# kahrendt/esp-audio-libs

Measured on NVIDIA B200. Metric: resampled output Msamples/s (4096 stereo streams, 256 taps), higher is better.
Workload: dtype f32

## Files before the change

esp-audio-libs_b200/csrc/kernels.hpp:

```cpp
#pragma once
#include <cuda.h>
#include <cuda_runtime.h>
#include <stddef.h>
#include <stdint.h>

#include "common.hpp"

namespace espb {

void count_launch();

struct PerDeviceOnce {
  bool done[64] = {};
  bool first() {
    int dev = 0;
    if (cudaGetDevice(&dev) != cudaSuccess || dev < 0 || dev >= 64)
      return true;
    const bool was = done[dev];
    done[dev] = true;
    return !was;
  }
};

struct ResampleParams {
  const float *xt;
  int64_t xt_rows;
  float *out;
  int64_t out_ss, out_cs, out_fs;
  float *out_tm;
  int64_t out_tm_rows;
  const float *G;
  const ChunkEntry *chunks;
  const int32_t *pass_chunk_begin;
  const OutEntry *outs;
  int n_series, channels, n_out, taps;
  int pass_first, pass_end, passes_per_cta, g_chunk_base;
  int out_vec;
  const int *ready;
  int ready_tiles, ready_target;
};
constexpr int kReadyTileRows = 32;
struct DirectInput {
  const float *in;
  int64_t in_ss;
  alignas(64) CUtensorMap map;
};
struct ResampleDirectParams {
  ResampleParams p;
  DirectInput d;
};
enum OutVec : int { kOutVecNone = 0, kOutVecPlanar = 1, kOutVecStereo = 2, kOutVecFrame4 = 3, kOutVecTimeMajor = 4 };

size_t resample_smem_bytes(int bpp, int chunk_rows, int g_row_floats = kGRowFloats);
size_t g_chunk_floats(int bpp, int chunk_rows, int g_row_floats = kGRowFloats);
cudaError_t launch_finalize(OutEntry *outs, int n, int n_filters, bool lowpass, bool interp, cudaStream_t stream);
cudaError_t launch_expand_schedule(const SchedSegment *segs, int n_segs, OutEntry *outs, int n, int n_filters,
                                   bool lowpass, bool interp, cudaStream_t stream);
cudaError_t launch_expand(const float *bank, const OutEntry *outs, const ChunkEntry *chunks, float *G,
                          int chunk_first, int n_chunks, int n_out, int taps, int bpp, int chunk_rows,
                          bool split_at_zero, cudaStream_t stream, int g_row_floats = kGRowFloats);
cudaError_t launch_resample(const ResampleParams &p, int bpp, int chunk_rows, bool exact, cudaStream_t stream,
                            const DirectInput *direct = nullptr, bool non_interpolating = false);
cudaError_t launch_resample_ni(const ResampleParams &q, int n_groups, int n_ctas_y, bool exact, bool tm,
                               cudaStream_t stream);
cudaError_t launch_resample_direct(const ResampleParams &p, const DirectInput &d, int n_groups, int n_ctas_y,
                                   bool exact, cudaStream_t stream);
cudaError_t launch_transpose(const float *in, int64_t in_ss, int64_t in_cs, int64_t in_fs, int channels, int n_series,
                             int n_in, float *xt, int64_t rows_cap, int row_first, int pad_rows,
                             cudaStream_t stream);
cudaError_t launch_transpose_flags(const float *in, int64_t in_ss, int64_t in_cs, int64_t in_fs, int channels,
                                   int n_series, int n_in, float *xt, int64_t rows_cap, int row_first, int pad_rows,
                                   int *ready, int ctas_per_sm, cudaStream_t stream, int *n_tiles);

struct FsGroupDesc {
  int64_t x_off;
  int64_t x_old_off;
  int64_t out_off;
  int64_t in_off;
  int32_t n_in, n_out;
  int32_t outs_begin;
  int32_t seg_begin, n_segs;
  int32_t carry_row;
};
cudaError_t launch_stage_small(const float *old_xt, int carry_row, int taps, const float *in, int64_t in_ss,
                               int64_t in_cs, int64_t in_fs, int channels, int n_series, int n_in, float *xt,
                               int64_t rows_cap, int pad_rows, cudaStream_t stream);
cudaError_t launch_transpose_ptrs(const float *const *planes_dev, int n_series, int n_in, float *xt, int64_t rows_cap,
                                  int row_first, int pad_rows, cudaStream_t stream);
cudaError_t launch_untranspose_ptrs(const float *tm, int64_t rows_cap, int row_first, int n_rows,
                                    float *const *planes_dev, int n_series, cudaStream_t stream);

struct FsParams {
  const float *x;
  int64_t x_fs;
  int x_row0;
  float *out;
  int64_t out_ss, out_cs, out_fs;
  float *out_tm;
  const float *bank_tr;
  const OutEntry *outs;
  int n_series, channels, n_out, taps;
  int kt, slice_floats;
  int q_per_out, x_tile_floats, out_vec, x_pitch, stages;
  const FsGroupDesc *groups;
};
struct FsGeometry {
  int sv, b, q;
  int outputs_per_cta;
};
constexpr int kFsMaxSeries = 32;
int fs_slice_taps(int taps, int filters);
size_t fs_slice_floats(int filters, int kt);
void fs_build_bank_slices(const float *bank, int taps, int filters, int kt, float *dst);
FsGeometry fs_geometry(int n_series);
size_t fs_smem_bytes(const FsGeometry &g, size_t slice_floats, int x_rows);
cudaError_t launch_resample_fs(const FsParams &p, const FsGeometry &g, int x_rows, bool exact, cudaStream_t stream,
                               int n_groups = 1);
cudaError_t launch_fsg_stage(const FsGroupDesc *groups, int n_groups, const float *old_buf, float *new_buf, int pitch,
                             int taps, const float *in, int64_t in_ss, int channels, int n_series, int max_rows,
                             cudaStream_t stream);
cudaError_t launch_expand_schedule_groups(const FsGroupDesc *groups, int n_groups, const SchedSegment *segs,
                                          OutEntry *outs, int max_n_out, int n_filters, bool lowpass, bool interp,
                                          cudaStream_t stream);

cudaError_t launch_q2f(const uint8_t *in, int64_t in_row_bytes, float *out, int64_t out_row_floats, int rows,
                       uint32_t row_samples, int bits, float gain_factor, cudaStream_t stream);
cudaError_t launch_f2q(const float *in, int64_t in_row_floats, uint8_t *out, int64_t out_row_bytes, int rows,
                       uint32_t row_samples, int bits, uint32_t *clipped, bool clipped_per_row, cudaStream_t stream);

int launch_pcm_to_tm(const uint8_t *in, int64_t in_row_bytes, int bits, float gain_factor, int channels, int n_series,
                     int n_frames, float *tm, int64_t rows_cap, int row_first, cudaStream_t stream, cudaError_t *err);
int launch_tm_to_pcm(const float *tm, int64_t rows_cap, int row_first, int n_frames, uint8_t *out,
                     int64_t out_row_bytes, int bits, int channels, int n_series, uint32_t *clipped_per_stream,
                     cudaStream_t stream, cudaError_t *err);
cudaError_t launch_transpose_from(const float *in, int64_t in_ss, int64_t in_cs, int64_t in_fs, int channels,
                                  int n_series, int n_in, float *xt, int64_t rows_cap, int row_first, int j_begin,
                                  int pad_rows, cudaStream_t stream);
cudaError_t launch_untranspose_from(const float *tm, int64_t rows_cap, int row_first, int j_begin, int n_rows,
                                    float *out, int64_t out_ss, int64_t out_cs, int64_t out_fs, int channels,
                                    int n_series, cudaStream_t stream);

struct BiquadParams {
  float a0, a1, a2, b1, b2;
  int first_order;
};
size_t biquad_block_state_floats(int n_series, int n_sections, int n_rows, int block_rows);
constexpr int kBiquadFewSeries = 32;
cudaError_t launch_biquad_cl(float *buf, int64_t ss, int64_t cs, int64_t fs, int channels, int n_series, int n_frames,
                             int n_sections, BiquadParams c, float *state, cudaStream_t stream);
cudaError_t launch_biquad_tm(const float *src, float *dst, int64_t rows_cap, int row_first, int n_rows, int n_series,
                             int n_sections, BiquadParams c, float *state ,
                             int block_rows, int warm_rows, cudaStream_t stream, float *blk_state = nullptr,
                             unsigned int *mismatches = nullptr, unsigned int *chain_broken = nullptr);
int launch_biquad_tm_pcm(float *buf, int64_t rows_cap, int row_first, int n_rows, int n_series, int n_sections,
                         BiquadParams c, float *state, uint8_t *out, int64_t out_row_bytes, int bits,
                         uint32_t *clipped_per_stream, cudaStream_t stream, cudaError_t *err);
cudaError_t launch_untranspose(const float *tm, int64_t rows_cap, int row_first, int n_rows, float *out,
                               int64_t out_ss, int64_t out_cs, int64_t out_fs, int channels, int n_series,
                               cudaStream_t stream);

cudaError_t launch_add_s16(const int16_t *a, const int16_t *b, int16_t *out, uint64_t n, int64_t s1, int64_t s2,
                           int64_t so, int shift, cudaStream_t stream);
cudaError_t launch_mulc_s16(const int16_t *a, int16_t *out, uint64_t n, int16_t c, int64_t si, int64_t so,
                            cudaStream_t stream);

cudaError_t launch_checksum(const uint32_t *words, uint64_t n, unsigned long long *sum_dev, cudaStream_t stream);
cudaError_t run_tile_probe(double *tflops);
cudaError_t run_fma_probe(double *tflops, double *clock_mhz, double *tflops_scalar, double *tflops_packed);

}
```

esp-audio-libs_b200/csrc/resample_device.cuh:

```cuda
#pragma once
#include <cuda.h>
#include <cuda_runtime.h>
#include <stdint.h>

#include "common.hpp"
#include "kernels.hpp"

namespace espb {
namespace {

constexpr int NB = kOutputsPerBlock;
constexpr int SGN = kSeriesPerRow;
constexpr uint32_t kPassDone = 1u << 9, kHistory = 1u << 10;
constexpr int RG = 4;

__device__ __forceinline__ uint32_t smem_u32(const void *p) { return (uint32_t) __cvta_generic_to_shared(p); }

__device__ __forceinline__ void mbar_init(uint64_t *bar, int count) {
  asm volatile("mbarrier.init.shared::cta.b64 [%0], %1;\n" ::"r"(smem_u32(bar)), "r"(count) : "memory");
}
__device__ __forceinline__ void mbar_expect_tx(uint64_t *bar, uint32_t bytes) {
  asm volatile("mbarrier.arrive.expect_tx.shared::cta.b64 _, [%0], %1;\n" ::"r"(smem_u32(bar)), "r"(bytes)
               : "memory");
}
__device__ __forceinline__ void mbar_wait(uint64_t *bar, uint32_t parity) {
  const uint32_t a = smem_u32(bar);
  asm volatile(
      "{\n"
      ".reg .pred p;\n"
      "WAIT_%=:\n"
      "mbarrier.try_wait.parity.shared::cta.b64 p, [%0], %1;\n"
      "@p bra DONE_%=;\n"
      "bra WAIT_%=;\n"
      "DONE_%=:\n"
      "}\n" ::"r"(a),
      "r"(parity)
      : "memory");
}
__device__ __forceinline__ void tma_bulk_g2s(void *dst_smem, const void *src, uint32_t bytes, uint64_t *bar) {
  asm volatile("cp.async.bulk.shared::cluster.global.mbarrier::complete_tx::bytes [%0], [%1], %2, [%3];\n" ::"r"(
                   smem_u32(dst_smem)),
               "l"(src), "r"(bytes), "r"(smem_u32(bar))
               : "memory");
}

__device__ __forceinline__ void tma_tensor2d_g2s(void *dst_smem, const CUtensorMap *map, int c0, int c1, uint64_t *bar) {
  asm volatile(
      "cp.async.bulk.tensor.2d.shared::cluster.global.tile.mbarrier::complete_tx::bytes [%0], [%1, {%2, %3}], [%4];\n" ::"r"(
          smem_u32(dst_smem)),
      "l"(map), "r"(c0), "r"(c1), "r"(smem_u32(bar))
      : "memory");
}

__device__ __forceinline__ void cp_async_16(void *dst_smem, const void *src) {
  asm volatile("cp.async.ca.shared.global [%0], [%1], 16;\n" ::"r"(smem_u32(dst_smem)), "l"(src) : "memory");
}
__device__ __forceinline__ void cp_async_wait_all() { asm volatile("cp.async.wait_all;\n" ::: "memory"); }

struct SwzTile {
  float *p;
  __device__ __forceinline__ static int unit(int row, int u) { return u ^ (((row >> 2) ^ ((row & 3) << 3)) & 31); }
  __device__ __forceinline__ float &at(int row, int col) const {
    return p[row * kSeriesPerRow + (unit(row, col >> 2) << 2) + (col & 3)];
  }
  __device__ __forceinline__ float4 &vec(int row, int u) const {
    return *reinterpret_cast<float4 *>(p + row * kSeriesPerRow + (unit(row, u) << 2));
  }
};

__device__ __forceinline__ int ld_acquire_gpu(const int *p) {
  int v;
  asm volatile("ld.acquire.gpu.global.s32 %0, [%1];\n" : "=r"(v) : "l"(p) : "memory");
  return v;
}
__device__ __forceinline__ void fence_proxy_async() { asm volatile("fence.proxy.async;\n" ::: "memory"); }
__device__ __forceinline__ void grid_launch_dependents() { asm volatile("griddepcontrol.launch_dependents;\n" ::: "memory"); }

__device__ __forceinline__ uint64_t l2_policy_evict_first() {
  uint64_t pol;
  asm volatile("createpolicy.fractional.L2::evict_first.b64 %0, 1.0;\n" : "=l"(pol));
  return pol;
}
__device__ __forceinline__ uint64_t l2_policy_evict_last() {
  uint64_t pol;
  asm volatile("createpolicy.fractional.L2::evict_last.b64 %0, 1.0;\n" : "=l"(pol));
  return pol;
}
__device__ __forceinline__ float4 ld_global_hint(const float4 *p, uint64_t pol) {
  float4 v;
  asm volatile("ld.global.nc.L1::no_allocate.L2::cache_hint.v4.f32 {%0, %1, %2, %3}, [%4], %5;\n"
               : "=f"(v.x), "=f"(v.y), "=f"(v.z), "=f"(v.w)
               : "l"(p), "l"(pol));
  return v;
}
__device__ __forceinline__ void st_global_hint(float4 *p, float4 v, uint64_t pol) {
  asm volatile("st.global.L2::cache_hint.v4.f32 [%0], {%1, %2, %3, %4}, %5;\n" ::"l"(p), "f"(v.x), "f"(v.y), "f"(v.z),
               "f"(v.w), "l"(pol)
               : "memory");
}
__device__ __forceinline__ void tma_bulk_g2s_hint(void *dst_smem, const void *src, uint32_t bytes, uint64_t *bar,
                                                  uint64_t pol) {
  asm volatile(
      "cp.async.bulk.shared::cluster.global.mbarrier::complete_tx::bytes.L2::cache_hint [%0], [%1], %2, [%3], %4;\n" ::"r"(
          smem_u32(dst_smem)),
      "l"(src), "r"(bytes), "r"(smem_u32(bar)), "l"(pol)
      : "memory");
}

__device__ __forceinline__ int smem_arrive(int *counter) {
  int old;
  asm volatile("atom.relaxed.cta.shared::cta.add.s32 %0, [%1], 1;\n" : "=r"(old) : "r"(smem_u32(counter)) : "memory");
  return old;
}

__device__ __forceinline__ float2 fma2(float2 g, float x, float2 acc) {
  return __ffma2_rn(g, make_float2(x, x), acc);
}

template <bool EXACT>
__device__ __forceinline__ float mac(float g, float x, float acc) {
  if (EXACT)
    return __fadd_rn(acc, __fmul_rn(g, x));
  return __fmaf_rn(g, x, acc);
}

}
}
```

esp-audio-libs_b200/csrc/resample_direct_kernel.cu:

```cuda
#include <cuda.h>
#include <cuda_runtime.h>
#include <stdint.h>
#include <stdio.h>
#include <stdlib.h>

#include "common.hpp"
#include "kernels.hpp"
#include "resample_device.cuh"

namespace espb {

template <int BPP, int NST, int CJ, bool EXACT, bool TMCAP, bool DIRECT>
__device__ __forceinline__ void resample_body(const ResampleParams &p, const DirectInput &din, unsigned char *smem_raw) {
  static_assert(!DIRECT || (CJ == 32 && !TMCAP), "direct input: 32-row chunks, caller-layout output");
  constexpr int NTHREADS = BPP * 32;
  constexpr int STAGES = NST;
  constexpr int MAXC = max_chunks_per_cta(BPP, CJ);
  static_assert(kMaxPassesPerCta * BPP * sizeof(int2) <= (size_t) NST * CJ * SGN * sizeof(float), "set-up table");
  constexpr int XS_STAGE = CJ * SGN;
  constexpr int GS_STAGE = CJ * BPP * kGRowFloats;
  constexpr uint32_t X_BYTES = XS_STAGE * sizeof(float), G_BYTES = GS_STAGE * sizeof(float);

  float *gs = reinterpret_cast<float *>(smem_raw);
  float *xs = gs + STAGES * GS_STAGE;
  uint64_t *full = reinterpret_cast<uint64_t *>(xs + STAGES * XS_STAGE);
  int *done = reinterpret_cast<int *>(full + STAGES);
  int32_t *jtab = reinterpret_cast<int32_t *>(done + 2 * STAGES);
  uint16_t *rtab = reinterpret_cast<uint16_t *>(jtab + MAXC);
  OutEntry *etab = reinterpret_cast<OutEntry *>(rtab + MAXC * BPP);
  int32_t *hdr = reinterpret_cast<int32_t *>(etab + BPP * NB);
  int2 *wtab = reinterpret_cast<int2 *>(smem_raw);

  const int tid = threadIdx.x, lane = tid & 31, warp = tid >> 5;
  const int group = blockIdx.x;
  const int T = p.taps;

  const int pass_first = p.pass_first + blockIdx.y * p.passes_per_cta;
  int pass_last = pass_first + p.passes_per_cta;
  if (pass_last > p.pass_end)
    pass_last = p.pass_end;
  const int chunk_first = p.pass_chunk_begin[pass_first], chunk_last = p.pass_chunk_begin[pass_last];
  const int n_chunks = __shfl_sync(0xffffffffu, chunk_last - chunk_first, 0);

  for (int i = tid; i < (pass_last - pass_first) * BPP; i += NTHREADS) {
    const int o0 = ((pass_first + i / BPP) * BPP + (i % BPP)) * NB;
    int2 w = make_int2(0, 0);
    if (o0 < p.n_out) {
      const int o1 = (o0 + NB <= p.n_out ? o0 + NB : p.n_out) - 1;
      w.x = p.outs[o0].ws;
      w.y = p.outs[o1].ws + T;
    }
    wtab[i] = w;
  }
  if (tid == 0) {
#pragma unroll
    for (int s = 0; s < STAGES; ++s) {
      mbar_init(&full[s], 1);
      done[s] = 0;
    }
    hdr[0] = chunk_first - p.g_chunk_base;
    asm volatile("fence.mbarrier_init.release.cluster;\n" ::: "memory");
  }
  __syncthreads();
  for (int i = tid; i < n_chunks; i += NTHREADS) {
    const ChunkEntry ce = p.chunks[chunk_first + i];
    const bool last_of_pass = (i + 1 == n_chunks) || (p.chunks[chunk_first + i + 1].pass != ce.pass);
    jtab[i] = ce.j_start;
#pragma unroll
    for (int w = 0; w < BPP; ++w) {
      const int2 win = wtab[(ce.pass - pass_first) * BPP + w];
      int r0 = win.x - ce.j_start, r1 = win.y - ce.j_start;
      r0 = r0 < 0 ? 0 : (r0 / RG);
      r1 = r1 > CJ ? CJ / RG : ((r1 + RG - 1) / RG);
      if (r0 > CJ / RG)
        r0 = CJ / RG;
      if (r1 < r0)
        r1 = r0;
      if (DIRECT && ce.j_start < 0) {
        const int lim = (-ce.j_start) / RG;
        r1 = r1 < lim ? r1 : lim;
        r0 = r0 < r1 ? r0 : r1;
      }
      rtab[i * BPP + w] = (uint16_t) (r0 | (r1 << 4) | (last_of_pass ? kPassDone : 0) |
                                      ((DIRECT && ce.j_start < 0) ? kHistory : 0));
    }
  }
  __syncthreads();

  auto issue_chunk = [&](int c) {
    const int st = c % STAGES;
    const float *xt_group = p.xt + (int64_t) blockIdx.x * p.xt_rows * SGN;
    mbar_expect_tx(&full[st], X_BYTES + G_BYTES);
    tma_bulk_g2s(gs + st * GS_STAGE, p.G + (size_t) (hdr[0] + c) * GS_STAGE, G_BYTES, &full[st]);
    const int j = jtab[c];
    if (DIRECT && j >= 0) {
      tma_tensor2d_g2s(xs + st * XS_STAGE, &din.map, 2 * j, (int) blockIdx.x * (SGN / 2), &full[st]);
      tma_tensor2d_g2s(xs + st * XS_STAGE + XS_STAGE / 2, &din.map, 2 * j + 32, (int) blockIdx.x * (SGN / 2), &full[st]);
    } else {
      tma_bulk_g2s(xs + st * XS_STAGE, xt_group + (int64_t) (j + T) * SGN, X_BYTES, &full[st]);
    }
  };
  if (tid == 0)
    for (int c = 0; c < STAGES && c < n_chunks; ++c)
      issue_chunk(c);

  float2 acc2[EXACT ? 1 : 4][EXACT ? 1 : NB];
  float acc1[EXACT ? 4 : 1][EXACT ? NB : 1][2];
  auto clear_acc = [&]() {
    if constexpr (EXACT) {
#pragma unroll
      for (int e = 0; e < 4; ++e)
#pragma unroll
        for (int n = 0; n < NB; ++n)
          acc1[e][n][0] = acc1[e][n][1] = 0.0f;
    } else {
#pragma unroll
      for (int e = 0; e < 4; ++e)
#pragma unroll
        for (int n = 0; n < NB; ++n)
          acc2[e][n] = make_float2(0.0f, 0.0f);
    }
  };
  clear_acc();

  int cur_pass = pass_first;
  uint32_t role_next = rtab[warp];
  for (int c = 0; c < n_chunks; ++c) {
    const int st = c % STAGES;
    const uint32_t role = role_next;
    const bool pass_done = (role & kPassDone) != 0;
    const int r0 = role & 15, r1 = (role >> 4) & 15;
    if (pass_done && lane < NB) {
      int o = (cur_pass * BPP + warp) * NB + lane;
      o = o < p.n_out ? o : p.n_out - 1;
      cp_async_16(&etab[warp * NB + lane], &p.outs[o]);
    }
    mbar_wait(&full[st], (uint32_t) ((c / STAGES) & 1));
    if constexpr (!DIRECT)
    {
      const float *xrow = xs + st * XS_STAGE + lane * 4;
      const float *grow = gs + st * GS_STAGE + warp * kGRowFloats;
      for (int jb = r0; jb < r1; ++jb) {
        const float *xb = xrow + jb * RG * SGN;
        const float *gb = grow + jb * RG * BPP * kGRowFloats;
#pragma unroll
        for (int jj = 0; jj < RG; ++jj) {
          const float4 xv = *reinterpret_cast<const float4 *>(xb + jj * SGN);
          if constexpr (EXACT) {
            const float4 *gp = reinterpret_cast<const float4 *>(gb + jj * BPP * kGRowFloats);
            const float4 g0 = gp[0], g1 = gp[1], g2 = gp[2], g3 = gp[3];
            const float x4[4] = {xv.x, xv.y, xv.z, xv.w};
            const float g16[16] = {g0.x, g0.y, g0.z, g0.w, g1.x, g1.y, g1.z, g1.w,
                                   g2.x, g2.y, g2.z, g2.w, g3.x, g3.y, g3.z, g3.w};
#pragma unroll
            for (int n = 0; n < NB; ++n)
#pragma unroll
              for (int e = 0; e < 4; ++e) {
                acc1[e][n][0] = mac<true>(g16[2 * n], x4[e], acc1[e][n][0]);
                acc1[e][n][1] = mac<true>(g16[2 * n + 1], x4[e], acc1[e][n][1]);
              }
          } else {
            const float4 *gp = reinterpret_cast<const float4 *>(gb + jj * BPP * kGRowFloats);
            const float4 g0 = gp[0], g1 = gp[1], g2 = gp[2], g3 = gp[3];
            const float x4[4] = {xv.x, xv.y, xv.z, xv.w};
            const float2 gg[NB] = {make_float2(g0.x, g0.y), make_float2(g0.z, g0.w), make_float2(g1.x, g1.y),
                                   make_float2(g1.z, g1.w), make_float2(g2.x, g2.y), make_float2(g2.z, g2.w),
                                   make_float2(g3.x, g3.y), make_float2(g3.z, g3.w)};
#pragma unroll
            for (int n = 0; n < NB; ++n)
#pragma unroll
              for (int e = 0; e < 4; ++e)
                acc2[e][n] = fma2(gg[n], x4[e], acc2[e][n]);
          }
        }
      }
    }
    else
    {
      auto row_update = [&](const float (&x4)[4], const float *grow_j) {
        const float4 *gp = reinterpret_cast<const float4 *>(grow_j);
        const float4 g0 = gp[0], g1 = gp[1], g2 = gp[2], g3 = gp[3];
        if constexpr (EXACT) {
          const float g16[16] = {g0.x, g0.y, g0.z, g0.w, g1.x, g1.y, g1.z, g1.w,
                                 g2.x, g2.y, g2.z, g2.w, g3.x, g3.y, g3.z, g3.w};
#pragma unroll
          for (int n = 0; n < NB; ++n)
#pragma unroll
            for (int e = 0; e < 4; ++e) {
              acc1[e][n][0] = mac<true>(g16[2 * n], x4[e], acc1[e][n][0]);
              acc1[e][n][1] = mac<true>(g16[2 * n + 1], x4[e], acc1[e][n][1]);
            }
        } else {
          const float2 gg[NB] = {make_float2(g0.x, g0.y), make_float2(g0.z, g0.w), make_float2(g1.x, g1.y),
// ... 195 lines not shown
```

esp-audio-libs_b200/csrc/resample_kernel.cu:

```cuda
#include <cuda_runtime.h>
#include <stdint.h>
#include <stdio.h>
#include <stdlib.h>

#include "common.hpp"
#include "kernels.hpp"
#include "resample_device.cuh"

namespace espb {


__global__ void __launch_bounds__(256)
    espb_finalize_kernel(OutEntry *__restrict__ outs, int n, float n_filters, int lowpass, int interp) {
  const int k = blockIdx.x * blockDim.x + threadIdx.x;
  if (k >= n)
    return;
  const float off = outs[k].w;
  const float fl = (float) (int) off;
  float frac = __fsub_rn(off, fl);
  OutEntry e;
  e.ws = outs[k].ws + (int32_t) fl;
  e.phase = 0;
  e.w = 0.0f;
  if (frac == 0.0f && !lowpass) {
// ... 327 lines not shown
                              float *__restrict__ xt, int64_t rows_cap, int row_first, int pad_rows) {
  __shared__ float tile[TR_ROWS][SGN + 1];
  const int g = blockIdx.x;
  const int j0 = blockIdx.y * TR_ROWS;
  const int tid = threadIdx.x;
  const int total_rows = n_in + pad_rows;
  for (int i = tid; i < SGN * TR_ROWS; i += 256) {
    const int sl = i / TR_ROWS, t = i - sl * TR_ROWS;
    const int q = g * SGN + sl, j = j0 + t;
    float v = 0.0f;
    if (q < n_series && j < n_in)
      v = __ldg(planes[q] + j);
    tile[t][sl] = v;
  }
  __syncthreads();
  float4 *dst = reinterpret_cast<float4 *>(xt + ((int64_t) g * rows_cap + row_first + j0) * SGN);
  for (int i = tid; i < TR_ROWS * (SGN / 4); i += 256) {
    const int t = i / (SGN / 4), c4 = i - t * (SGN / 4);
    if (j0 + t < total_rows)
      dst[i] = make_float4(tile[t][c4 * 4], tile[t][c4 * 4 + 1], tile[t][c4 * 4 + 2], tile[t][c4 * 4 + 3]);
  }
}

__global__ void __launch_bounds__(256)
    espb_untranspose_ptr_kernel(const float *__restrict__ tm, int64_t rows_cap, int row_first, int n_rows,
                                float *const *__restrict__ planes, int n_series) {
  __shared__ float tile[TR_ROWS][SGN + 1];
  const int g = blockIdx.x;
  const int j0 = blockIdx.y * TR_ROWS;
  const int tid = threadIdx.x;
  const float *src = tm + ((int64_t) g * rows_cap + row_first + j0) * SGN;
  for (int i = tid; i < TR_ROWS * SGN; i += 256) {
    const int t = i / SGN, sl = i - t * SGN;
    tile[t][sl] = (j0 + t < n_rows) ? __ldg(src + i) : 0.0f;
  }
  __syncthreads();
  for (int i = tid; i < SGN * TR_ROWS; i += 256) {
    const int sl = i / TR_ROWS, t = i - sl * TR_ROWS;
    const int q = g * SGN + sl, j = j0 + t;
    if (q < n_series && j < n_rows)
      planes[q][j] = tile[t][sl];
  }
}

template <int CH, bool PLANAR>
__global__ void __launch_bounds__(TF_THREADS)
    espb_untranspose_fast_kernel(const float *__restrict__ tm, int64_t rows_cap, int row_first, float *__restrict__ out,
                                 int64_t out_ss, int64_t out_cs, int channels, int n_series) {
  __shared__ __align__(16) float tile_s[TF_ROWS * SGN];
  const SwzTile tile{tile_s};
  const int g = blockIdx.x;
  const int j0 = blockIdx.y * TF_ROWS;
  const int tid = threadIdx.x;
  const float4 *src = reinterpret_cast<const float4 *>(tm + ((int64_t) g * rows_cap + row_first + j0) * SGN);
  constexpr int UNITS = SGN / CH;
  constexpr int V_PER_UNIT = TF_ROWS * CH / 4;
  const int units = (n_series - g * SGN + 3) / 4 < SGN / 4 ? (n_series - g * SGN + 3) / 4 : SGN / 4;
  const int runs_here = (units * 4 + CH - 1) / CH < UNITS ? (units * 4 + CH - 1) / CH : UNITS;
#pragma unroll 4
  for (int i = tid; i < TF_ROWS * (SGN / 4); i += TF_THREADS) {
    const int t = i / (SGN / 4), c4 = i % (SGN / 4);
    if (c4 < units)
      tile.vec(t, c4) = __ldg(src + i);
  }
  __syncthreads();
#pragma unroll 4
  for (int v = tid; v < runs_here * V_PER_UNIT; v += TF_THREADS) {
    const int unit = v / V_PER_UNIT, off4 = v % V_PER_UNIT;
    const int q0 = g * SGN + unit * CH;
    if (q0 >= n_series)
      continue;
    float *dst;
    if (PLANAR) {
      const int st = q0 / channels, ch = q0 - st * channels;
      dst = out + (int64_t) st * out_ss + (int64_t) ch * out_cs + j0;
    } else {
      dst = out + (int64_t) (q0 / CH) * out_ss + (int64_t) j0 * CH;
    }
    const int e0 = off4 * 4;
    float x[4];
#pragma unroll
    for (int k = 0; k < 4; ++k) {
      const int e = e0 + k;
      x[k] = tile.at(e / CH, unit * CH + (e % CH));
    }
    reinterpret_cast<float4 *>(dst)[off4] = make_float4(x[0], x[1], x[2], x[3]);
  }
}

__global__ void __launch_bounds__(256)
    espb_untranspose_kernel(const float *__restrict__ tm, int64_t rows_cap, int row_first, int j_begin, int n_rows,
                            float *__restrict__ out, int64_t out_ss, int64_t out_cs, int64_t out_fs, int channels,
                            int n_series) {
  __shared__ float tile[TR_ROWS][SGN + 1];
  const int g = blockIdx.x;
  const int j0 = j_begin + blockIdx.y * TR_ROWS;
  const int tid = threadIdx.x;
  const float *src = tm + ((int64_t) g * rows_cap + row_first + j0) * SGN;
  for (int i = tid; i < TR_ROWS * SGN; i += 256) {
    const int t = i / SGN, sl = i - t * SGN;
    tile[t][sl] = (j0 + t < n_rows) ? __ldg(src + i) : 0.0f;
  }
  __syncthreads();
  const int mapping = (out_fs == 1) ? 0 : ((out_cs == 1 && out_fs == channels && SGN % channels == 0) ? 1 : 2);
  for (int i = tid; i < SGN * TR_ROWS; i += 256) {
    int sl, t;
    if (mapping == 0) {
      sl = i / TR_ROWS;
      t = i - sl * TR_ROWS;
    } else if (mapping == 1) {
      const int per = TR_ROWS * channels;
      const int stl = i / per, r = i - stl * per;
      t = r / channels;
      sl = stl * channels + (r - t * channels);
    } else {
      t = i / SGN;
      sl = i - t * SGN;
    }
    const int q = g * SGN + sl, j = j0 + t;
    if (q < n_series && j < n_rows) {
      const int st = q / channels, ch = q - st * channels;
      out[(int64_t) st * out_ss + (int64_t) ch * out_cs + (int64_t) j * out_fs] = tile[t][sl];
    }
  }
}

__device__ __forceinline__ void out_store4(float4 *p, float4 v) { *p = v; }

template <int BPP, int NST, int CJ, bool EXACT, bool TMCAP>
__global__ void __launch_bounds__(BPP * 32, 16 / BPP) espb_resample_kernel(const ResampleParams p) {
  constexpr int NTHREADS = BPP * 32;
  constexpr int STAGES = NST;
  constexpr int MAXC = max_chunks_per_cta(BPP, CJ);
  static_assert(kMaxPassesPerCta * BPP * sizeof(int2) <= (size_t) NST * CJ * SGN * sizeof(float), "set-up table");
  constexpr int XS_STAGE = CJ * SGN;
  constexpr int GS_STAGE = CJ * BPP * kGRowFloats;
  constexpr uint32_t X_BYTES = XS_STAGE * sizeof(float), G_BYTES = GS_STAGE * sizeof(float);

  extern __shared__ __align__(128) unsigned char smem_raw[];
  float *gs = reinterpret_cast<float *>(smem_raw);
  float *xs = gs + STAGES * GS_STAGE;
  uint64_t *full = reinterpret_cast<uint64_t *>(xs + STAGES * XS_STAGE);
  int *done = reinterpret_cast<int *>(full + STAGES);
  int32_t *jtab = reinterpret_cast<int32_t *>(done + 2 * STAGES);
  uint16_t *rtab = reinterpret_cast<uint16_t *>(jtab + MAXC);
  OutEntry *etab = reinterpret_cast<OutEntry *>(rtab + MAXC * BPP);
  int32_t *hdr = reinterpret_cast<int32_t *>(etab + BPP * NB);
  int2 *wtab = reinterpret_cast<int2 *>(smem_raw);

  const int tid = threadIdx.x, lane = tid & 31, warp = tid >> 5;
  const int group = blockIdx.x;
  const int T = p.taps;

  const int pass_first = p.pass_first + blockIdx.y * p.passes_per_cta;
  int pass_last = pass_first + p.passes_per_cta;
  if (pass_last > p.pass_end)
    pass_last = p.pass_end;
  const int chunk_first = p.pass_chunk_begin[pass_first], chunk_last = p.pass_chunk_begin[pass_last];
  const int n_chunks = __shfl_sync(0xffffffffu, chunk_last - chunk_first, 0);

  for (int i = tid; i < (pass_last - pass_first) * BPP; i += NTHREADS) {
    const int o0 = ((pass_first + i / BPP) * BPP + (i % BPP)) * NB;
    int2 w = make_int2(0, 0);
    if (o0 < p.n_out) {
      const int o1 = (o0 + NB <= p.n_out ? o0 + NB : p.n_out) - 1;
      w.x = p.outs[o0].ws;
      w.y = p.outs[o1].ws + T;
    }
    wtab[i] = w;
  }
  if (tid == 0) {
#pragma unroll
    for (int s = 0; s < STAGES; ++s) {
      mbar_init(&full[s], 1);
      done[s] = 0;
    }
    hdr[0] = chunk_first - p.g_chunk_base;
    asm volatile("fence.mbarrier_init.release.cluster;\n" ::: "memory");
  }
  __syncthreads();
  for (int i = tid; i < n_chunks; i += NTHREADS) {
    const ChunkEntry ce = p.chunks[chunk_first + i];
    const bool last_of_pass = (i + 1 == n_chunks) || (p.chunks[chunk_first + i + 1].pass != ce.pass);
    jtab[i] = ce.j_start;
#pragma unroll
    for (int w = 0; w < BPP; ++w) {
      const int2 win = wtab[(ce.pass - pass_first) * BPP + w];
      int r0 = win.x - ce.j_start, r1 = win.y - ce.j_start;
      r0 = r0 < 0 ? 0 : (r0 / RG);
      r1 = r1 > CJ ? CJ / RG : ((r1 + RG - 1) / RG);
      if (r0 > CJ / RG)
        r0 = CJ / RG;
      if (r1 < r0)
        r1 = r0;
      rtab[i * BPP + w] = (uint16_t) (r0 | (r1 << 4) | (last_of_pass ? kPassDone : 0));
    }
  }
  __syncthreads();

  auto issue_chunk = [&](int c) {
    const int st = c % STAGES;
    const float *xt_group = p.xt + (int64_t) blockIdx.x * p.xt_rows * SGN;
    mbar_expect_tx(&full[st], X_BYTES + G_BYTES);
    tma_bulk_g2s(gs + st * GS_STAGE, p.G + (size_t) (hdr[0] + c) * GS_STAGE, G_BYTES, &full[st]);
    tma_bulk_g2s(xs + st * XS_STAGE, xt_group + (int64_t) (jtab[c] + T) * SGN, X_BYTES, &full[st]);
  };
  if (p.ready != nullptr && n_chunks > 0) {
    const int j_hi = jtab[n_chunks - 1] + CJ - 1;
    if (j_hi >= 0) {
      const int j_lo = jtab[0];
      const int y_lo = j_lo > 0 ? j_lo / kReadyTileRows : 0;
      int y_hi = j_hi / kReadyTileRows;
      y_hi = y_hi < p.ready_tiles ? y_hi : p.ready_tiles - 1;
      for (int y = y_lo + tid; y <= y_hi; y += NTHREADS) {
        const long long t0 = clock64();
        while (ld_acquire_gpu(p.ready + y) < p.ready_target) {
          __nanosleep(200);
          if (clock64() - t0 > (4ll << 31))
            __trap();
        }
      }
    }
    __syncthreads();
    fence_proxy_async();
  }
  if (tid == 0)
    for (int c = 0; c < STAGES && c < n_chunks; ++c)
      issue_chunk(c);

  float2 acc2[EXACT ? 1 : 4][EXACT ? 1 : NB];
  float acc1[EXACT ? 4 : 1][EXACT ? NB : 1][2];
  auto clear_acc = [&]() {
    if constexpr (EXACT) {
#pragma unroll
      for (int e = 0; e < 4; ++e)
#pragma unroll
        for (int n = 0; n < NB; ++n)
          acc1[e][n][0] = acc1[e][n][1] = 0.0f;
    } else {
#pragma unroll
      for (int e = 0; e < 4; ++e)
#pragma unroll
        for (int n = 0; n < NB; ++n)
          acc2[e][n] = make_float2(0.0f, 0.0f);
    }
  };
  clear_acc();

  int cur_pass = pass_first;
  uint32_t role_next = rtab[warp];
  for (int c = 0; c < n_chunks; ++c) {
    const int st = c % STAGES;
    const uint32_t role = role_next;
    const bool pass_done = (role & kPassDone) != 0;
    const int r0 = role & 15, r1 = (role >> 4) & 15;
    if (pass_done && lane < NB) {
      int o = (cur_pass * BPP + warp) * NB + lane;
      o = o < p.n_out ? o : p.n_out - 1;
      cp_async_16(&etab[warp * NB + lane], &p.outs[o]);
    }
    mbar_wait(&full[st], (uint32_t) ((c / STAGES) & 1));
    {
      const float *xrow = xs + st * XS_STAGE + lane * 4;
      const float *grow = gs + st * GS_STAGE + warp * kGRowFloats;
      for (int jb = r0; jb < r1; ++jb) {
        const float *xb = xrow + jb * RG * SGN;
        const float *gb = grow + jb * RG * BPP * kGRowFloats;
#pragma unroll
        for (int jj = 0; jj < RG; ++jj) {
          const float4 xv = *reinterpret_cast<const float4 *>(xb + jj * SGN);
          if constexpr (EXACT) {
            const float4 *gp = reinterpret_cast<const float4 *>(gb + jj * BPP * kGRowFloats);
            const float4 g0 = gp[0], g1 = gp[1], g2 = gp[2], g3 = gp[3];
            const float x4[4] = {xv.x, xv.y, xv.z, xv.w};
            const float g16[16] = {g0.x, g0.y, g0.z, g0.w, g1.x, g1.y, g1.z, g1.w,
                                   g2.x, g2.y, g2.z, g2.w, g3.x, g3.y, g3.z, g3.w};
#pragma unroll
            for (int n = 0; n < NB; ++n)
#pragma unroll
              for (int e = 0; e < 4; ++e) {
                acc1[e][n][0] = mac<true>(g16[2 * n], x4[e], acc1[e][n][0]);
                acc1[e][n][1] = mac<true>(g16[2 * n + 1], x4[e], acc1[e][n][1]);
              }
          } else {
            const float4 *gp = reinterpret_cast<const float4 *>(gb + jj * BPP * kGRowFloats);
            const float4 g0 = gp[0], g1 = gp[1], g2 = gp[2], g3 = gp[3];
            const float x4[4] = {xv.x, xv.y, xv.z, xv.w};
            const float2 gg[NB] = {make_float2(g0.x, g0.y), make_float2(g0.z, g0.w), make_float2(g1.x, g1.y),
                                   make_float2(g1.z, g1.w), make_float2(g2.x, g2.y), make_float2(g2.z, g2.w),
                                   make_float2(g3.x, g3.y), make_float2(g3.z, g3.w)};
#pragma unroll
            for (int n = 0; n < NB; ++n)
#pragma unroll
              for (int e = 0; e < 4; ++e)
                acc2[e][n] = fma2(gg[n], x4[e], acc2[e][n]);
          }
        }
      }
    }

    role_next = rtab[(c + 1) * BPP + warp];
    __syncwarp();
    if (lane == 0) {
      if (smem_arrive(&done[st]) == BPP - 1) {
        done[st] = 0;
        if (c + STAGES < n_chunks)
          issue_chunk(c + STAGES);
      }
    }

// ... 258 lines not shown
                               int64_t rows_cap, int pad_rows, cudaStream_t stream) {
  const int n_groups = (n_series + SGN - 1) / SGN;
  if (n_groups <= 0)
    return cudaSuccess;
  const int hist_tiles = (taps + TR_ROWS - 1) / TR_ROWS;
  dim3 grid(n_groups, hist_tiles + (n_in + pad_rows + TR_ROWS - 1) / TR_ROWS);
  espb_stage_small_kernel<<<grid, 256, 0, stream>>>(old_xt, carry_row, taps, hist_tiles, in, in_ss, in_cs, in_fs,
                                                    channels, n_series, n_in, xt, rows_cap, pad_rows);
  count_launch();
  return cudaGetLastError();
}

cudaError_t launch_transpose_ptrs(const float *const *planes_dev, int n_series, int n_in, float *xt, int64_t rows_cap,
                                  int row_first, int pad_rows, cudaStream_t stream) {
  const int n_groups = (n_series + SGN - 1) / SGN;
  if (n_groups <= 0 || n_in + pad_rows <= 0)
    return cudaSuccess;
  dim3 grid(n_groups, (n_in + pad_rows + TR_ROWS - 1) / TR_ROWS);
  espb_transpose_ptr_kernel<<<grid, 256, 0, stream>>>(planes_dev, n_series, n_in, xt, rows_cap, row_first, pad_rows);
  count_launch();
  return cudaGetLastError();
}

cudaError_t launch_untranspose_ptrs(const float *tm, int64_t rows_cap, int row_first, int n_rows,
                                    float *const *planes_dev, int n_series, cudaStream_t stream) {
  const int n_groups = (n_series + SGN - 1) / SGN;
  if (n_groups <= 0 || n_rows <= 0)
    return cudaSuccess;
  dim3 grid(n_groups, (n_rows + TR_ROWS - 1) / TR_ROWS);
  espb_untranspose_ptr_kernel<<<grid, 256, 0, stream>>>(tm, rows_cap, row_first, n_rows, planes_dev, n_series);
  count_launch();
  return cudaGetLastError();
}

cudaError_t launch_transpose_from(const float *in, int64_t in_ss, int64_t in_cs, int64_t in_fs, int channels,
                                  int n_series, int n_in, float *xt, int64_t rows_cap, int row_first, int j_begin,
                                  int pad_rows, cudaStream_t stream) {
  const int n_groups = (n_series + SGN - 1) / SGN;
  const int rest = n_in + pad_rows - j_begin;
  if (n_groups <= 0 || rest <= 0)
    return cudaSuccess;
  dim3 grid(n_groups, (rest + TR_ROWS - 1) / TR_ROWS);
  espb_transpose_kernel<<<grid, 256, 0, stream>>>(in, in_ss, in_cs, in_fs, channels, n_series, n_in, xt, rows_cap,
                                                  row_first, j_begin, pad_rows);
  count_launch();
  return cudaGetLastError();
}

cudaError_t launch_untranspose_from(const float *tm, int64_t rows_cap, int row_first, int j_begin, int n_rows,
                                    float *out, int64_t out_ss, int64_t out_cs, int64_t out_fs, int channels,
                                    int n_series, cudaStream_t stream) {
  const int n_groups = (n_series + SGN - 1) / SGN;
  const int rest = n_rows - j_begin;
  if (n_groups <= 0 || rest <= 0)
    return cudaSuccess;
  dim3 grid(n_groups, (rest + TR_ROWS - 1) / TR_ROWS);
  espb_untranspose_kernel<<<grid, 256, 0, stream>>>(tm, rows_cap, row_first, j_begin, n_rows, out, out_ss, out_cs,
                                                    out_fs, channels, n_series);
  count_launch();
  return cudaGetLastError();
}

cudaError_t launch_untranspose(const float *tm, int64_t rows_cap, int row_first, int n_rows, float *out,
                               int64_t out_ss, int64_t out_cs, int64_t out_fs, int channels, int n_series,
                               cudaStream_t stream) {
  const int n_groups = (n_series + SGN - 1) / SGN;
  if (n_groups <= 0 || n_rows <= 0)
    return cudaSuccess;
  int fast_rows = 0;
  const bool aligned = ((uintptr_t) out % 16 == 0) && (out_ss % 4 == 0);
  const bool interleaved = (out_cs == 1 && out_fs == channels);
  const bool planar = (out_fs == 1) && (out_cs % 4 == 0);
  if (aligned && n_rows >= TF_ROWS) {
    dim3 grid(n_groups, n_rows / TF_ROWS);
    bool done = true;
    if (interleaved && channels == 1)
      espb_untranspose_fast_kernel<1, false><<<grid, TF_THREADS, 0, stream>>>(tm, rows_cap, row_first, out, out_ss,
                                                                              out_cs, channels, n_series);
    else if (interleaved && channels == 2)
      espb_untranspose_fast_kernel<2, false><<<grid, TF_THREADS, 0, stream>>>(tm, rows_cap, row_first, out, out_ss,
                                                                              out_cs, channels, n_series);
    else if (interleaved && channels == 4)
      espb_untranspose_fast_kernel<4, false><<<grid, TF_THREADS, 0, stream>>>(tm, rows_cap, row_first, out, out_ss,
                                                                              out_cs, channels, n_series);
    else if (interleaved && channels == 8)
      espb_untranspose_fast_kernel<8, false><<<grid, TF_THREADS, 0, stream>>>(tm, rows_cap, row_first, out, out_ss,
                                                                              out_cs, channels, n_series);
    else if (planar)
      espb_untranspose_fast_kernel<1, true><<<grid, TF_THREADS, 0, stream>>>(tm, rows_cap, row_first, out, out_ss,
                                                                             out_cs, channels, n_series);
    else
      done = false;
    if (done) {
      count_launch();
      fast_rows = (n_rows / TF_ROWS) * TF_ROWS;
      cudaError_t e = cudaGetLastError();
      if (e != cudaSuccess)
        return e;
    }
  }
  const int rest = n_rows - fast_rows;
  if (rest > 0) {
    dim3 grid(n_groups, (rest + TR_ROWS - 1) / TR_ROWS);
    espb_untranspose_kernel<<<grid, 256, 0, stream>>>(tm, rows_cap, row_first, fast_rows, n_rows, out, out_ss, out_cs,
                                                      out_fs, channels, n_series);
    count_launch();
  }
  return cudaGetLastError();
}

template <int BPP, int NST, int CJ, bool EXACT, bool TMCAP>
static cudaError_t launch_resample_t(const ResampleParams &p, int n_groups, int n_ctas_y, cudaStream_t stream) {
  const size_t smem = resample_smem_bytes(BPP, CJ);
  static PerDeviceOnce once;
  if (once.first()) {
    cudaError_t e = cudaFuncSetAttribute(espb_resample_kernel<BPP, NST, CJ, EXACT, TMCAP>,
                                         cudaFuncAttributeMaxDynamicSharedMemorySize, (int) smem);
    if (e != cudaSuccess)
      return e;
    e = cudaFuncSetAttribute(espb_resample_kernel<BPP, NST, CJ, EXACT, TMCAP>, cudaFuncAttributePreferredSharedMemoryCarveout,
                             (int) cudaSharedmemCarveoutMaxShared);
    if (e != cudaSuccess)
      return e;
    if (getenv("ESPB_DEBUG")) {
      int nb = 0;
      cudaOccupancyMaxActiveBlocksPerMultiprocessor(&nb, espb_resample_kernel<BPP, NST, CJ, EXACT, TMCAP>, BPP * 32, smem);
      cudaFuncAttributes fa;
      cudaFuncGetAttributes(&fa, espb_resample_kernel<BPP, NST, CJ, EXACT, TMCAP>);
      fprintf(stderr, "[espb] resample<%d,%d,%d,%d,%d>: smem %zu B, %d regs, occupancy %d CTA/SM\n", BPP, NST, CJ,
              (int) EXACT, (int) TMCAP, smem, fa.numRegs, nb);
    }
  }
  dim3 grid(n_groups, n_ctas_y);
  if (p.ready != nullptr) {
    cudaLaunchConfig_t cfg = {};
    cfg.gridDim = grid;
    cfg.blockDim = dim3(BPP * 32);
    cfg.dynamicSmemBytes = smem;
    cfg.stream = stream;
    cudaLaunchAttribute attr[1];
    attr[0].id = cudaLaunchAttributeProgrammaticStreamSerialization;
    attr[0].val.programmaticStreamSerializationAllowed = 1;
    cfg.attrs = attr;
    cfg.numAttrs = 1;
    cudaError_t e = cudaLaunchKernelEx(&cfg, espb_resample_kernel<BPP, NST, CJ, EXACT, TMCAP>, p);
    count_launch();
    return e != cudaSuccess ? e : cudaGetLastError();
  }
  espb_resample_kernel<BPP, NST, CJ, EXACT, TMCAP><<<grid, BPP * 32, smem, stream>>>(p);
  count_launch();
  return cudaGetLastError();
}

cudaError_t launch_resample(const ResampleParams &p, int bpp, int chunk_rows, bool exact, cudaStream_t stream,
                            const DirectInput *direct, bool non_interpolating) {
  const int n_groups = (p.n_series + SGN - 1) / SGN;
  const int n_passes = p.pass_end - p.pass_first;
  if (n_groups <= 0 || n_passes <= 0)
    return cudaSuccess;
  const int n_ctas_y = (n_passes + p.passes_per_cta - 1) / p.passes_per_cta;
  const bool tm = p.out_tm != nullptr;
  ResampleParams q = p;
  q.out_vec = tm ? kOutVecTimeMajor : kOutVecNone;
  if (!tm && (uintptr_t) p.out % 16 == 0 && p.out_ss % 4 == 0) {
    if (p.out_fs == 1 && (p.out_cs % 4 == 0 || p.channels == 1))
      q.out_vec = kOutVecPlanar;
    else if (p.out_cs == 1 && p.out_fs == p.channels && p.channels == 2)
      q.out_vec = kOutVecStereo;
    else if (p.out_cs == 1 && p.out_fs == p.channels && p.channels % 4 == 0)
      q.out_vec = kOutVecFrame4;
  }
#define ESPB_LAUNCH(BPP_, NST_, CJ_)                                                               \
  (exact ? (tm ? launch_resample_t<BPP_, NST_, CJ_, true, true>(q, n_groups, n_ctas_y, stream)     \
               : launch_resample_t<BPP_, NST_, CJ_, true, false>(q, n_groups, n_ctas_y, stream))   \
         : (tm ? launch_resample_t<BPP_, NST_, CJ_, false, true>(q, n_groups, n_ctas_y, stream)    \
               : launch_resample_t<BPP_, NST_, CJ_, false, false>(q, n_groups, n_ctas_y, stream)))
  if (non_interpolating) {
    if (bpp != 4 || chunk_rows != 32 || direct)
      return cudaErrorInvalidValue;
    return launch_resample_ni(q, n_groups, n_ctas_y, exact, tm, stream);
  }
  if (direct) {
    if (bpp != 4 || chunk_rows != 32 || tm)
      return cudaErrorInvalidValue;
    return launch_resample_direct(q, *direct, n_groups, n_ctas_y, exact, stream);
  }
  if (bpp == 8 && chunk_rows == 32)
    return ESPB_LAUNCH(8, 3, 32);
  if (bpp == 4 && chunk_rows == 32)
    return ESPB_LAUNCH(4, 2, 32);
  if (bpp == 8 && chunk_rows == 16)
    return ESPB_LAUNCH(8, 6, 16);
  if (bpp == 4 && chunk_rows == 16)
    return ESPB_LAUNCH(4, 4, 16);
  if (bpp == 4 && chunk_rows == 24)
    return ESPB_LAUNCH(4, 3, 24);
  if (bpp == 4 && chunk_rows == 36)
    return ESPB_LAUNCH(4, 2, 36);
#undef ESPB_LAUNCH
  return cudaErrorInvalidValue;
}

}
```

esp-audio-libs_b200/csrc/resample_ni_kernel.cu:

```cuda
#include <cuda_runtime.h>
#include <stdint.h>
#include <stdio.h>
#include <stdlib.h>

#include "common.hpp"
#include "kernels.hpp"
#include "resample_device.cuh"

namespace espb {

template <int BPP, int NST, int CJ, bool EXACT, bool TMCAP>
__global__ void __launch_bounds__(BPP * 32, 16 / BPP) espb_resample_ni_kernel(const ResampleParams p) {
  constexpr int GRF = kGRowFloatsNI;
  constexpr int WB = kNiBlocksPerWarp;
  constexpr int PB = BPP * WB;
  constexpr int NO = NB * WB;
  constexpr int NTHREADS = BPP * 32;
  constexpr int STAGES = NST;
  constexpr int MAXC = max_chunks_per_cta(BPP, CJ);
  static_assert(kMaxPassesPerCta * BPP * sizeof(int2) <= (size_t) NST * CJ * SGN * sizeof(float), "set-up table");
  constexpr int XS_STAGE = CJ * SGN;
  constexpr int GS_STAGE = CJ * PB * GRF;
  constexpr uint32_t X_BYTES = XS_STAGE * sizeof(float), G_BYTES = GS_STAGE * sizeof(float);

  extern __shared__ __align__(128) unsigned char smem_raw[];
  float *gs = reinterpret_cast<float *>(smem_raw);
  float *xs = gs + STAGES * GS_STAGE;
  uint64_t *full = reinterpret_cast<uint64_t *>(xs + STAGES * XS_STAGE);
  int *done = reinterpret_cast<int *>(full + STAGES);
  int32_t *jtab = reinterpret_cast<int32_t *>(done + 2 * STAGES);
  uint16_t *rtab = reinterpret_cast<uint16_t *>(jtab + MAXC);
  OutEntry *etab = reinterpret_cast<OutEntry *>(rtab + MAXC * BPP);
  int32_t *hdr = reinterpret_cast<int32_t *>(etab + BPP * NO);
  int2 *wtab = reinterpret_cast<int2 *>(smem_raw);

  const int tid = threadIdx.x, lane = tid & 31, warp = tid >> 5;
  const int group = blockIdx.x;
  const int T = p.taps;

  const int pass_first = p.pass_first + blockIdx.y * p.passes_per_cta;
  int pass_last = pass_first + p.passes_per_cta;
  if (pass_last > p.pass_end)
    pass_last = p.pass_end;
  const int chunk_first = p.pass_chunk_begin[pass_first], chunk_last = p.pass_chunk_begin[pass_last];
  const int n_chunks = __shfl_sync(0xffffffffu, chunk_last - chunk_first, 0);

  for (int i = tid; i < (pass_last - pass_first) * BPP; i += NTHREADS) {
    const int o0 = ((pass_first + i / BPP) * PB + (i % BPP) * WB) * NB;
    int2 w = make_int2(0, 0);
    if (o0 < p.n_out) {
      const int o1 = (o0 + NO <= p.n_out ? o0 + NO : p.n_out) - 1;
      w.x = p.outs[o0].ws;
      w.y = p.outs[o1].ws + T;
    }
    wtab[i] = w;
  }
  if (tid == 0) {
#pragma unroll
    for (int s = 0; s < STAGES; ++s) {
      mbar_init(&full[s], 1);
      done[s] = 0;
    }
    hdr[0] = chunk_first - p.g_chunk_base;
    asm volatile("fence.mbarrier_init.release.cluster;\n" ::: "memory");
  }
  __syncthreads();
  for (int i = tid; i < n_chunks; i += NTHREADS) {
    const ChunkEntry ce = p.chunks[chunk_first + i];
    const bool last_of_pass = (i + 1 == n_chunks) || (p.chunks[chunk_first + i + 1].pass != ce.pass);
    jtab[i] = ce.j_start;
#pragma unroll
    for (int w = 0; w < BPP; ++w) {
      const int2 win = wtab[(ce.pass - pass_first) * BPP + w];
      int r0 = win.x - ce.j_start, r1 = win.y - ce.j_start;
      r0 = r0 < 0 ? 0 : (r0 / RG);
      r1 = r1 > CJ ? CJ / RG : ((r1 + RG - 1) / RG);
      if (r0 > CJ / RG)
        r0 = CJ / RG;
      if (r1 < r0)
        r1 = r0;
      rtab[i * BPP + w] = (uint16_t) (r0 | (r1 << 4) | (last_of_pass ? kPassDone : 0));
    }
  }
  __syncthreads();

  auto issue_chunk = [&](int c) {
    const int st = c % STAGES;
    const float *xt_group = p.xt + (int64_t) blockIdx.x * p.xt_rows * SGN;
    mbar_expect_tx(&full[st], X_BYTES + G_BYTES);
    tma_bulk_g2s(gs + st * GS_STAGE, p.G + (size_t) (hdr[0] + c) * GS_STAGE, G_BYTES, &full[st]);
    tma_bulk_g2s(xs + st * XS_STAGE, xt_group + (int64_t) (jtab[c] + T) * SGN, X_BYTES, &full[st]);
  };
  if (p.ready != nullptr && n_chunks > 0) {
    const int j_hi = jtab[n_chunks - 1] + CJ - 1;
    if (j_hi >= 0) {
      const int j_lo = jtab[0];
      const int y_lo = j_lo > 0 ? j_lo / kReadyTileRows : 0;
      int y_hi = j_hi / kReadyTileRows;
      y_hi = y_hi < p.ready_tiles ? y_hi : p.ready_tiles - 1;
      for (int y = y_lo + tid; y <= y_hi; y += NTHREADS) {
        const long long t0 = clock64();
        while (ld_acquire_gpu(p.ready + y) < p.ready_target) {
          __nanosleep(200);
          if (clock64() - t0 > (4ll << 31))
            __trap();
        }
      }
    }
    __syncthreads();
    fence_proxy_async();
  }
  if (tid == 0)
    for (int c = 0; c < STAGES && c < n_chunks; ++c)
      issue_chunk(c);

  float acc[EXACT ? 4 : 1][EXACT ? NO : 1];
  float2 accp[EXACT ? 1 : 4][EXACT ? 1 : NO / 2];
  auto clear_acc = [&]() {
    if constexpr (EXACT) {
#pragma unroll
      for (int e = 0; e < 4; ++e)
#pragma unroll
        for (int n = 0; n < NO; ++n)
          acc[e][n] = 0.0f;
    } else {
#pragma unroll
      for (int e = 0; e < 4; ++e)
#pragma unroll
        for (int m = 0; m < NO / 2; ++m)
          accp[e][m] = make_float2(0.0f, 0.0f);
    }
  };
  clear_acc();

  int cur_pass = pass_first;
  uint32_t role_next = rtab[warp];
  for (int c = 0; c < n_chunks; ++c) {
    const int st = c % STAGES;
    const uint32_t role = role_next;
    const bool pass_done = (role & kPassDone) != 0;
    const int r0 = role & 15, r1 = (role >> 4) & 15;
    if (pass_done && lane < NO) {
      int o = (cur_pass * PB + warp * WB) * NB + lane;
      o = o < p.n_out ? o : p.n_out - 1;
      cp_async_16(&etab[warp * NO + lane], &p.outs[o]);
    }
    mbar_wait(&full[st], (uint32_t) ((c / STAGES) & 1));
    {
      const float *xrow = xs + st * XS_STAGE + lane * 4;
      const float *grow = gs + st * GS_STAGE + warp * WB * GRF;
      for (int jb = r0; jb < r1; ++jb) {
        const float *xb = xrow + jb * RG * SGN;
        const float *gb = grow + jb * RG * PB * GRF;
#pragma unroll
        for (int jj = 0; jj < RG; ++jj) {
          const float4 xv = *reinterpret_cast<const float4 *>(xb + jj * SGN);
          const float4 *gp = reinterpret_cast<const float4 *>(gb + jj * PB * GRF);
          const float4 g0 = gp[0], g1 = gp[1], g2 = gp[2], g3 = gp[3];
          const float x4[4] = {xv.x, xv.y, xv.z, xv.w};
          if constexpr (EXACT) {
            const float g16[NO] = {g0.x, g0.y, g0.z, g0.w, g1.x, g1.y, g1.z, g1.w,
                                   g2.x, g2.y, g2.z, g2.w, g3.x, g3.y, g3.z, g3.w};
#pragma unroll
            for (int n = 0; n < NO; ++n)
#pragma unroll
              for (int e = 0; e < 4; ++e)
                acc[e][n] = mac<true>(g16[n], x4[e], acc[e][n]);
          } else {
            const float2 gg[NO / 2] = {make_float2(g0.x, g0.y), make_float2(g0.z, g0.w), make_float2(g1.x, g1.y),
                                       make_float2(g1.z, g1.w), make_float2(g2.x, g2.y), make_float2(g2.z, g2.w),
                                       make_float2(g3.x, g3.y), make_float2(g3.z, g3.w)};
#pragma unroll
            for (int m = 0; m < NO / 2; ++m)
#pragma unroll
              for (int e = 0; e < 4; ++e)
                accp[e][m] = fma2(gg[m], x4[e], accp[e][m]);
          }
        }
      }
    }

    role_next = rtab[(c + 1) * BPP + warp];
    __syncwarp();
    if (lane == 0) {
      if (smem_arrive(&done[st]) == BPP - 1) {
        done[st] = 0;
        if (c + STAGES < n_chunks)
          issue_chunk(c + STAGES);
      }
    }

    if (pass_done) {
      cp_async_wait_all();
      __syncwarp();
      const int series0 = group * SGN + lane * 4;
#pragma unroll
// ... 138 lines not shown
```

Measured before the change: 52980.

## Split trailing passes into single-pass CTAs to balance the tail wave

Changes the CTA-to-pass mapping so most CTAs still process passes_per_cta passes, while a tail of about two waves' worth of CTAs each handle a single pass. The goal is to shrink the load imbalance at the end of the grid, where a few long CTAs would otherwise leave SMs idle. The cost is more CTAs, each repeating its own set-up and pipeline prologue, plus a device attribute query on every launch. All three resample kernels share the new mapping helper.

```diff
diff --git a/esp-audio-libs_b200/csrc/kernels.hpp b/esp-audio-libs_b200/csrc/kernels.hpp
--- a/esp-audio-libs_b200/csrc/kernels.hpp
+++ b/esp-audio-libs_b200/csrc/kernels.hpp
@@ -38,6 +38,7 @@
   int out_vec;
   const int *ready;
   int ready_tiles, ready_target;
+  int long_rows;
 };
 constexpr int kReadyTileRows = 32;
 struct DirectInput {
diff --git a/esp-audio-libs_b200/csrc/resample_device.cuh b/esp-audio-libs_b200/csrc/resample_device.cuh
--- a/esp-audio-libs_b200/csrc/resample_device.cuh
+++ b/esp-audio-libs_b200/csrc/resample_device.cuh
@@ -117,6 +117,18 @@
   return __ffma2_rn(g, make_float2(x, x), acc);
 }
 
+__device__ __forceinline__ void cta_passes(const ResampleParams &p, int y, int &first, int &last) {
+  if (y < p.long_rows) {
+    first = p.pass_first + y * p.passes_per_cta;
+    last = first + p.passes_per_cta;
+    if (last > p.pass_end)
+      last = p.pass_end;
+  } else {
+    first = p.pass_first + p.long_rows * p.passes_per_cta + (y - p.long_rows);
+    last = first + 1;
+  }
+}
+
 template <bool EXACT>
 __device__ __forceinline__ float mac(float g, float x, float acc) {
   if (EXACT)
diff --git a/esp-audio-libs_b200/csrc/resample_direct_kernel.cu b/esp-audio-libs_b200/csrc/resample_direct_kernel.cu
--- a/esp-audio-libs_b200/csrc/resample_direct_kernel.cu
+++ b/esp-audio-libs_b200/csrc/resample_direct_kernel.cu
@@ -35,10 +35,8 @@
   const int group = blockIdx.x;
   const int T = p.taps;
 
-  const int pass_first = p.pass_first + blockIdx.y * p.passes_per_cta;
-  int pass_last = pass_first + p.passes_per_cta;
-  if (pass_last > p.pass_end)
-    pass_last = p.pass_end;
+  int pass_first, pass_last;
+  cta_passes(p, blockIdx.y, pass_first, pass_last);
   const int chunk_first = p.pass_chunk_begin[pass_first], chunk_last = p.pass_chunk_begin[pass_last];
   const int n_chunks = __shfl_sync(0xffffffffu, chunk_last - chunk_first, 0);
 
diff --git a/esp-audio-libs_b200/csrc/resample_kernel.cu b/esp-audio-libs_b200/csrc/resample_kernel.cu
--- a/esp-audio-libs_b200/csrc/resample_kernel.cu
+++ b/esp-audio-libs_b200/csrc/resample_kernel.cu
@@ -503,10 +503,8 @@
   const int group = blockIdx.x;
   const int T = p.taps;
 
-  const int pass_first = p.pass_first + blockIdx.y * p.passes_per_cta;
-  int pass_last = pass_first + p.passes_per_cta;
-  if (pass_last > p.pass_end)
-    pass_last = p.pass_end;
+  int pass_first, pass_last;
+  cta_passes(p, blockIdx.y, pass_first, pass_last);
   const int chunk_first = p.pass_chunk_begin[pass_first], chunk_last = p.pass_chunk_begin[pass_last];
   const int n_chunks = __shfl_sync(0xffffffffu, chunk_last - chunk_first, 0);
 
@@ -1071,15 +1069,30 @@
   return cudaGetLastError();
 }
 
+constexpr long kTailWaves = 2;
+
 cudaError_t launch_resample(const ResampleParams &p, int bpp, int chunk_rows, bool exact, cudaStream_t stream,
                             const DirectInput *direct, bool non_interpolating) {
   const int n_groups = (p.n_series + SGN - 1) / SGN;
   const int n_passes = p.pass_end - p.pass_first;
   if (n_groups <= 0 || n_passes <= 0)
     return cudaSuccess;
-  const int n_ctas_y = (n_passes + p.passes_per_cta - 1) / p.passes_per_cta;
+  const int ppc = p.passes_per_cta;
+  int long_rows = (n_passes + ppc - 1) / ppc, n_ctas_y = long_rows;
+  if (ppc > 1) {
+    int sms = 148, dev = 0;
+    if (cudaGetDevice(&dev) == cudaSuccess)
+      cudaDeviceGetAttribute(&sms, cudaDevAttrMultiProcessorCount, dev);
+    const long slots = (long) sms * (16 / bpp);
+    long tail = (kTailWaves * slots + n_groups - 1) / n_groups;
+    if (tail > n_passes / 2)
+      tail = n_passes / 2;
+    long_rows = (int) ((n_passes - tail) / ppc);
+    n_ctas_y = long_rows + (n_passes - long_rows * ppc);
+  }
   const bool tm = p.out_tm != nullptr;
   ResampleParams q = p;
+  q.long_rows = long_rows;
   q.out_vec = tm ? kOutVecTimeMajor : kOutVecNone;
   if (!tm && (uintptr_t) p.out % 16 == 0 && p.out_ss % 4 == 0) {
     if (p.out_fs == 1 && (p.out_cs % 4 == 0 || p.channels == 1))
diff --git a/esp-audio-libs_b200/csrc/resample_ni_kernel.cu b/esp-audio-libs_b200/csrc/resample_ni_kernel.cu
--- a/esp-audio-libs_b200/csrc/resample_ni_kernel.cu
+++ b/esp-audio-libs_b200/csrc/resample_ni_kernel.cu
@@ -38,10 +38,8 @@
   const int group = blockIdx.x;
   const int T = p.taps;
 
-  const int pass_first = p.pass_first + blockIdx.y * p.passes_per_cta;
-  int pass_last = pass_first + p.passes_per_cta;
-  if (pass_last > p.pass_end)
-    pass_last = p.pass_end;
+  int pass_first, pass_last;
+  cta_passes(p, blockIdx.y, pass_first, pass_last);
   const int chunk_first = p.pass_chunk_begin[pass_first], chunk_last = p.pass_chunk_begin[pass_last];
   const int n_chunks = __shfl_sync(0xffffffffu, chunk_last - chunk_first, 0);
 
```

After: 52860, median of 6. No clear change (-0.2%).
